# andrewjong/SwapNet

Hardware: NVIDIA H100
Metric: images/sec (G+D fwd+bwd) warp-stage 512x512 (higher is better)
Workload: dtype fp16/bf16-split x3 tensor-core products, fp32 accumulate (fp32-faithful)

## Files before the change

swapnet_b200/csrc/gemm_tc.cu:

```cuda
#include "common.cuh"
#include "plan.h"

namespace {

constexpr int kBlockM = 128;
constexpr int kTileRing = 4;
constexpr int kTileBytes = 16384;
constexpr int kConsumerWarps = 8;
constexpr int kProducerWarp = kConsumerWarps;
constexpr int kThreads = (kConsumerWarps + 1) * 32;

template <int NSPLIT>
struct Cfg {
  static constexpr int kPlanes = NSPLIT == 3 ? 2 : 1;
  static constexpr int kStages = NSPLIT == 3 ? 3 : 6;
  static constexpr int kStageBytes = kPlanes * 2 * kTileBytes;
  static constexpr int kSmemBytes = kStages * kStageBytes + 1024;
};

__device__ __forceinline__ float apply_act(float v, int act) {
  if (act == SN_ACT_TANH) return tanhf(v);
  return v;
}

__device__ __forceinline__ float quad_col_sum(float v) {
  v += __shfl_xor_sync(0xffffffffu, v, 4);
  v += __shfl_xor_sync(0xffffffffu, v, 8);
  v += __shfl_xor_sync(0xffffffffu, v, 16);
  return v;
}

template <int NSPLIT, int CW, int BN, bool F16>
__global__ void __launch_bounds__(kThreads, 1)
tap_gemm_kernel(const __grid_constant__ TapGemmParams p, const int m_tiles, const int n_tiles, const int total_tiles) {
  const auto tile_coords = [&](int tile, int& mt, int& nt, int& z) {
    nt = tile % n_tiles;
    const int rest = tile / n_tiles;
    mt = rest % m_tiles;
    z = rest / m_tiles;
  };
  using C = Cfg<NSPLIT>;
  extern __shared__ uint8_t smem_raw[];
  __shared__ __align__(8) uint64_t full_bar[C::kStages];
  __shared__ __align__(8) uint64_t empty_bar[C::kStages];
  __shared__ __align__(8) uint64_t tr_full[kTileRing];
  __shared__ __align__(8) uint64_t tr_empty[kTileRing];
  __shared__ int tile_ring[kTileRing];

  const uint32_t smem_base = (smem_u32(smem_raw) + 1023u) & ~1023u;
  uint8_t* smem = smem_raw + (smem_base - smem_u32(smem_raw));
  const int warp = threadIdx.x >> 5;
  const int lane = threadIdx.x & 31;

  constexpr int cw = CW;
  constexpr int tps = 64 / cw;
  const int tpp = p.ntaps / p.nphase;
  const int k_iters = cw == 64 ? tpp * p.chunks : tpp / tps;

  if (threadIdx.x == 0) {
    for (int s = 0; s < C::kStages; ++s) {
      mbar_init(&full_bar[s], 1);
      mbar_init(&empty_bar[s], 2);
    }
    for (int r = 0; r < kTileRing; ++r) {
      mbar_init(&tr_full[r], 1);
      mbar_init(&tr_empty[r], kConsumerWarps);
    }
    mbar_fence_init();
  }
  if (warp == kProducerWarp && lane == 0) {
    for (int pl = 0; pl < C::kPlanes; ++pl) {
      tma_prefetch_desc(&p.tmA[pl]);
      tma_prefetch_desc(&p.tmB[pl]);
    }
  }
  __syncthreads();

  if (warp == kProducerWarp) {
    if (lane == 0) {
      const uint32_t stage_tx = C::kPlanes * (p.a_rows * 128 + p.block_n * 128);
      uint32_t it = 0, tcount = 0;
      for (int tile = blockIdx.x;; ++tcount) {
        const int next = tile < total_tiles ? (int)gridDim.x + atomicAdd(p.tile_counter, 1) : total_tiles;
        const uint32_t slot = tcount % kTileRing, rph = (tcount / kTileRing) & 1;
        mbar_wait(&tr_empty[slot], rph ^ 1);
        tile_ring[slot] = tile < total_tiles ? tile : -1;
        mbar_arrive(&tr_full[slot]);
        if (tile >= total_tiles) break;
        int mt, nt, z;
        tile_coords(tile, mt, nt, z);
        const int ncol0 = nt * p.block_n;
        const int tap0 = z * tpp;
        const int w0 = (mt % p.tiles_w) * p.tw;
        const int h0 = ((mt / p.tiles_w) % p.tiles_h) * p.th;
        const int n0 = (mt / (p.tiles_w * p.tiles_h)) * p.nb;
        for (int k = 0; k < k_iters; ++k, ++it) {
          const uint32_t s = it % C::kStages;
          const uint32_t ph = (it / C::kStages) & 1;
          mbar_wait(&empty_bar[s], ph ^ 1);
          mbar_expect_tx(&full_bar[s], stage_tx);
          uint8_t* st = smem + s * C::kStageBytes;
          if (cw == 64) {
            const int t = k / p.chunks;
            const int ch = k - t * p.chunks;
            const TapDesc tap = p.taps[tap0 + t];
            if (p.a_merged) {
              tma_load_5d(&p.tmA[0], &full_bar[s], st, tap.c_off + ch * 64, w0 + tap.dw, h0 + tap.dh, n0, 0);
            } else {
#pragma unroll
              for (int pl = 0; pl < C::kPlanes; ++pl)
                tma_load_5d(&p.tmA[pl], &full_bar[s], st + pl * kTileBytes, tap.c_off + ch * 64,
                            w0 + tap.dw, tap.hp, h0 + tap.dh, n0);
            }
            if (p.b_merged) {
              tma_load_3d(&p.tmB[0], &full_bar[s], st + C::kPlanes * kTileBytes, tap.kb_off + ch * 64, ncol0, 0);
            } else {
#pragma unroll
              for (int pl = 0; pl < C::kPlanes; ++pl)
                tma_load_2d(&p.tmB[pl], &full_bar[s], st + (C::kPlanes + pl) * kTileBytes,
                            tap.kb_off + ch * 64, ncol0);
            }
          } else {
            constexpr int sub = 128 * cw * 2;
#pragma unroll
            for (int j = 0; j < tps; ++j) {
              const TapDesc tap = p.taps[tap0 + k * tps + j];
#pragma unroll
              for (int pl = 0; pl < C::kPlanes; ++pl)
                tma_load_5d(&p.tmA[pl], &full_bar[s], st + pl * kTileBytes + j * sub, tap.c_off,
                            w0 + tap.dw, tap.hp, h0 + tap.dh, n0);
            }
            const int kb = p.taps[tap0 + k * tps].kb_off;
            if (p.b_merged) {
              tma_load_3d(&p.tmB[0], &full_bar[s], st + C::kPlanes * kTileBytes, kb, ncol0, 0);
            } else {
#pragma unroll
              for (int pl = 0; pl < C::kPlanes; ++pl)
                tma_load_2d(&p.tmB[pl], &full_bar[s], st + (C::kPlanes + pl) * kTileBytes, kb, ncol0);
            }
          }
        }
        tile = next;
      }
    }
  } else {
    const int wg = warp >> 2;
    const int quad = lane & 3;
    const int row0 = wg * 64 + (warp & 3) * 16 + (lane >> 2);
    int w_i[2], h_i[2], n_i[2];
#pragma unroll
    for (int h = 0; h < 2; ++h) {
      const int row = row0 + 8 * h;
      w_i[h] = row % p.tw;
      h_i[h] = (row / p.tw) % p.th;
      n_i[h] = row / (p.tw * p.th);
    }
    const float oscale = p.b_scale ? p.b_scale[1] : 1.f;
    float acc[BN / 2];
    uint32_t it = 0;
    for (uint32_t tcount = 0;; ++tcount) {
      const uint32_t slot = tcount % kTileRing, rph = (tcount / kTileRing) & 1;
      mbar_wait(&tr_full[slot], rph);
      const int tile = tile_ring[slot];
      __syncwarp();
      if (lane == 0) mbar_arrive(&tr_empty[slot]);
      if (tile < 0) break;
      for (int k = 0; k < k_iters; ++k, ++it) {
        const uint32_t s = it % C::kStages;
        const uint32_t ph = (it / C::kStages) & 1;
        mbar_wait(&full_bar[s], ph);
        const uint32_t st = smem_base + s * C::kStageBytes;
        constexpr uint32_t a_layout = cw >= 64 ? 1u : (cw == 32 ? 2u : 3u);
        constexpr uint32_t a_sbo = 8u * cw * 2u;
        const uint32_t a_row0 = (uint32_t)wg * 64u * cw * 2u;
        const uint64_t a_hi = gmma_smem_desc(st + a_row0, 16, a_sbo, a_layout);
        const uint64_t b_hi = gmma_smem_desc(st + C::kPlanes * kTileBytes, 16, 1024);
        const uint64_t a_lo = gmma_smem_desc(st + p.a_lo_off + a_row0, 16, a_sbo, a_layout);
        const uint64_t b_lo = gmma_smem_desc(st + C::kPlanes * kTileBytes + p.b_lo_off, 16, 1024);
        constexpr uint32_t sub16 = (uint32_t)(128 * cw * 2) >> 4;
        wgmma_fence();
#pragma unroll
        for (int kk = 0; kk < 4; ++kk) {
          const uint64_t badv = (uint64_t)(kk * 2);
          const uint64_t aadv = (uint64_t)(((kk * 16) / cw) * sub16 + (((kk * 16) % cw) >> 3));
          Wgmma<BN, F16>::template mma<0, 0>(acc, a_hi + aadv, b_hi + badv, (k | kk) != 0);
          if (NSPLIT == 3) {
            Wgmma<BN, F16>::template mma<0, 0>(acc, a_lo + aadv, b_hi + badv, 1);
            Wgmma<BN, F16>::template mma<0, 0>(acc, a_hi + aadv, b_lo + badv, 1);
          }
        }
        wgmma_commit();
        wgmma_wait<0>();
        wgmma_fence_acc(acc);
        if ((threadIdx.x & 127) == 0) mbar_arrive(&empty_bar[s]);
      }

      int mt, nt, z;
      tile_coords(tile, mt, nt, z);
      const int ncol0 = nt * p.block_n;
      const int ph_h = p.nphase == 4 ? (z >> 1) : 0, ph_w = p.nphase == 4 ? (z & 1) : 0;
      int gw[2], gh[2], gn[2];
      bool valid[2];
      float* optr[2];
#pragma unroll
      for (int h = 0; h < 2; ++h) {
        gw[h] = (mt % p.tiles_w) * p.tw + w_i[h];
        gh[h] = ((mt / p.tiles_w) % p.tiles_h) * p.th + h_i[h];
        gn[h] = (mt / (p.tiles_w * p.tiles_h)) * p.nb + n_i[h];
        valid[h] = (row0 + 8 * h < p.a_rows) && (gw[h] < p.m_w) && (gh[h] < p.m_h) && (gn[h] < p.m_n);
        optr[h] = p.out + (long long)gn[h] * p.out_sn + (long long)(gh[h] * p.omh + p.ooh + ph_h) * p.out_sh +
                  (long long)(gw[h] * p.omw + p.oow + ph_w) * p.out_sw + ncol0;
      }
#pragma unroll
      for (int i = 0; i < BN / 8; ++i) {
        const int c = 8 * i + 2 * quad;
        if (BN > 16 && 8 * i >= p.block_n) break;
        if (p.stack_slot) {
#pragma unroll
          for (int h = 0; h < 2; ++h) {
            if (!valid[h]) continue;
#pragma unroll
            for (int e = 0; e < 2; ++e) {
              const int col = ncol0 + c + e;
              const int ph = col / p.stack_slot, ch = col - ph * p.stack_slot;
              if (ph < 4 && ch < p.stack_c) {
                float v = acc[4 * i + 2 * h + e] * oscale;
                if (p.bias) v += p.bias[ch];
                float* o = p.out + (long long)gn[h] * p.out_sn + (long long)(gh[h] * p.omh + (ph >> 1)) * p.out_sh +
                           (long long)(gw[h] * p.omw + (ph & 1)) * p.out_sw + ch;
                *o = apply_act(v, p.act);
              }
            }
          }
        } else if (p.stats) {
          if (ncol0 + 8 * i >= p.n_valid) continue;
          float v[2][2];
#pragma unroll
          for (int h = 0; h < 2; ++h) {
#pragma unroll
            for (int e = 0; e < 2; ++e) {
              float t = acc[4 * i + 2 * h + e] * oscale;
              if (p.bias) t += p.bias[ncol0 + c + e];
              v[h][e] = valid[h] ? t : 0.f;
            }
            if (valid[h]) *reinterpret_cast<float2*>(optr[h] + c) = make_float2(v[h][0], v[h][1]);
          }
          const float s0 = quad_col_sum(v[0][0] + v[1][0]);
          const float s1 = quad_col_sum(v[0][1] + v[1][1]);
          const float q0 = quad_col_sum(v[0][0] * v[0][0] + v[1][0] * v[1][0]);
          const float q1 = quad_col_sum(v[0][1] * v[0][1] + v[1][1] * v[1][1]);
          if (lane < 4) {
            const int tn = (mt / (p.tiles_w * p.tiles_h)) * p.nb;
            double* sp = p.stats + ((long long)tn * p.n_valid + ncol0 + c) * 2;
            atomicAdd(sp, (double)s0);
            atomicAdd(sp + 1, (double)q0);
            atomicAdd(sp + 2, (double)s1);
            atomicAdd(sp + 3, (double)q1);
          }
        } else {
#pragma unroll
          for (int h = 0; h < 2; ++h) {
            if (!valid[h]) continue;
            float v0 = acc[4 * i + 2 * h] * oscale, v1 = acc[4 * i + 2 * h + 1] * oscale;
            const int col = ncol0 + c;
            if (p.vec4 && col + 1 < p.n_valid) {
              if (p.bias) {
                const float2 bb = *reinterpret_cast<const float2*>(p.bias + col);
                v0 += bb.x; v1 += bb.y;
              }
              *reinterpret_cast<float2*>(optr[h] + c) = make_float2(apply_act(v0, p.act), apply_act(v1, p.act));
            } else {
              if (col < p.n_valid) optr[h][c] = apply_act(p.bias ? v0 + p.bias[col] : v0, p.act);
              if (col + 1 < p.n_valid) optr[h][c + 1] = apply_act(p.bias ? v1 + p.bias[col + 1] : v1, p.act);
            }
          }
        }
      }
    }
  }

  __syncthreads();
  if (threadIdx.x == 0) {
    __threadfence();
    if (atomicAdd(p.tile_counter + 1, 1) == (int)gridDim.x - 1) {
      p.tile_counter[0] = 0;
      p.tile_counter[1] = 0;
      __threadfence();
    }
  }
}

// ... 129 lines not shown
        const int row = row0 + 8 * h;
        if (row >= p.rows_valid) continue;
        float* orow = p.out + (long long)row * p.s_row;
#pragma unroll
        for (int i = 0; i < BN / 8; ++i) {
#pragma unroll
          for (int e = 0; e < 2; ++e) {
            const int c = 8 * i + 2 * quad + e;
            const float v = acc[4 * i + 2 * h + e];
            if (!grouped) {
              const int col = ncol0 + c;
              if (c < p.block_n && col < p.cols_valid) atomicAdd(orow + p.tap_off[tap_i] + (long long)col * p.s_col, v);
            } else {
              const int b = c / ycw;
              const int cbase = c - b * ycw;
              if (b < gsize && cbase < p.cols_valid)
                atomicAdd(orow + p.tap_off[tap_i + b] + (long long)cbase * p.s_col, v);
            }
          }
        }
      }
    }
  }
}

}

typedef CUresult (*PFN_encodeTiled)(CUtensorMap*, CUtensorMapDataType, cuuint32_t, void*,
                                    const cuuint64_t*, const cuuint64_t*, const cuuint32_t*,
                                    const cuuint32_t*, CUtensorMapInterleave, CUtensorMapSwizzle,
                                    CUtensorMapL2promotion, CUtensorMapFloatOOBfill);

static PFN_encodeTiled get_encode_fn() {
  static PFN_encodeTiled fn = nullptr;
  if (!fn) {
    void* ptr = nullptr;
    cudaDriverEntryPointQueryResult qres;
    cudaError_t e = cudaGetDriverEntryPoint("cuTensorMapEncodeTiled", &ptr, cudaEnableDefault, &qres);
    if (e != cudaSuccess || qres != cudaDriverEntryPointSuccess || !ptr) return nullptr;
    fn = reinterpret_cast<PFN_encodeTiled>(ptr);
  }
  return fn;
}

int sn_make_act_map(CUtensorMap* tm, const void* base, int N, int H, int W, int C, int pitch,
                    int parity, int box_w, int box_h, int box_n, int chunk = 64, long long plane_stride = 0) {
  PFN_encodeTiled enc = get_encode_fn();
  SN_REQUIRE(enc != nullptr, "cuTensorMapEncodeTiled driver entry point unavailable");
  SN_REQUIRE(pitch % 8 == 0 && ((uintptr_t)base % 16) == 0,
             "activation plane needs 16-B aligned base and pitch %% 8 == 0 (pitch=%d)", pitch);
  SN_REQUIRE(box_w >= 1 && box_h >= 1 && box_n >= 1 && box_w <= 256 && box_h <= 256 && box_n <= 256,
             "bad TMA box %d x %d x %d", box_w, box_h, box_n);
  cuuint64_t dims[5];
  cuuint64_t strides[4];
  const cuuint64_t e = 2;
  cuuint32_t box[5] = {(cuuint32_t)chunk, (cuuint32_t)box_w, 1, (cuuint32_t)box_h, (cuuint32_t)box_n};
  if (plane_stride > 0) {
    SN_REQUIRE(plane_stride % 16 == 0, "merged planes: 16-B aligned plane stride");
    if (!parity) {
      dims[0] = C; dims[1] = W; dims[2] = H; dims[3] = N; dims[4] = 2;
      strides[0] = (cuuint64_t)pitch * e;
      strides[1] = (cuuint64_t)W * pitch * e;
    } else {
      SN_REQUIRE(H % 2 == 0 && W % 2 == 0, "parity view needs even H, W (got %d x %d)", H, W);
      dims[0] = (cuuint64_t)(W + 1) * pitch + C; dims[1] = W / 2; dims[2] = H / 2; dims[3] = N; dims[4] = 2;
      strides[0] = (cuuint64_t)2 * pitch * e;
      strides[1] = (cuuint64_t)2 * W * pitch * e;
    }
    strides[2] = (cuuint64_t)H * W * pitch * e;
    strides[3] = (cuuint64_t)plane_stride;
    box[2] = (cuuint32_t)box_h; box[3] = (cuuint32_t)box_n; box[4] = 2;
  } else if (!parity) {
    dims[0] = C; dims[1] = W; dims[2] = 1; dims[3] = H; dims[4] = N;
    strides[0] = (cuuint64_t)pitch * e;
    strides[1] = (cuuint64_t)W * pitch * e;
    strides[2] = (cuuint64_t)W * pitch * e;
    strides[3] = (cuuint64_t)H * W * pitch * e;
  } else {
    SN_REQUIRE(H % 2 == 0 && W % 2 == 0, "parity view needs even H, W (got %d x %d)", H, W);
    dims[0] = (cuuint64_t)pitch + C; dims[1] = W / 2; dims[2] = 2; dims[3] = H / 2; dims[4] = N;
    strides[0] = (cuuint64_t)2 * pitch * e;
    strides[1] = (cuuint64_t)W * pitch * e;
    strides[2] = (cuuint64_t)2 * W * pitch * e;
    strides[3] = (cuuint64_t)H * W * pitch * e;
  }
  SN_REQUIRE(chunk == 64 || chunk == 32 || chunk == 16, "row chunk must be 64, 32 or 16 channels (got %d)", chunk);
  cuuint32_t estr[5] = {1, 1, 1, 1, 1};
  const CUtensorMapSwizzle swz = chunk == 64 ? CU_TENSOR_MAP_SWIZZLE_128B
                                 : chunk == 32 ? CU_TENSOR_MAP_SWIZZLE_64B : CU_TENSOR_MAP_SWIZZLE_32B;
  CUresult r = enc(tm, CU_TENSOR_MAP_DATA_TYPE_BFLOAT16, 5, const_cast<void*>(base), dims, strides,
                   box, estr, CU_TENSOR_MAP_INTERLEAVE_NONE, swz,
                   CU_TENSOR_MAP_L2_PROMOTION_L2_256B, CU_TENSOR_MAP_FLOAT_OOB_FILL_NONE);
  SN_REQUIRE(r == CUDA_SUCCESS,
             "cuTensorMapEncodeTiled(act) failed: %d (N=%d H=%d W=%d C=%d pitch=%d parity=%d box=%dx%dx%d)",
             (int)r, N, H, W, C, pitch, parity, box_w, box_h, box_n);
  return SN_OK;
}

int sn_make_weight_map(CUtensorMap* tm, const void* base, int rows, long long k_total, int box_rows,
                       long long plane_stride = 0) {
  PFN_encodeTiled enc = get_encode_fn();
  SN_REQUIRE(enc != nullptr, "cuTensorMapEncodeTiled driver entry point unavailable");
  SN_REQUIRE(k_total % 64 == 0 && ((uintptr_t)base % 16) == 0, "packed weights need K %% 64 == 0");
  cuuint64_t dims[3] = {(cuuint64_t)k_total, (cuuint64_t)rows, 2};
  cuuint64_t strides[2] = {(cuuint64_t)k_total * 2, (cuuint64_t)plane_stride};
  cuuint32_t box[3] = {64, (cuuint32_t)box_rows, 2};
  cuuint32_t estr[3] = {1, 1, 1};
  CUresult r = enc(tm, CU_TENSOR_MAP_DATA_TYPE_BFLOAT16, plane_stride > 0 ? 3 : 2, const_cast<void*>(base), dims, strides,
                   box, estr, CU_TENSOR_MAP_INTERLEAVE_NONE, CU_TENSOR_MAP_SWIZZLE_128B,
                   CU_TENSOR_MAP_L2_PROMOTION_L2_256B, CU_TENSOR_MAP_FLOAT_OOB_FILL_NONE);
  SN_REQUIRE(r == CUDA_SUCCESS, "cuTensorMapEncodeTiled(weights) failed: %d (rows=%d K=%lld box_rows=%d)",
             (int)r, rows, k_total, box_rows);
  return SN_OK;
}

static void pick_patch(int m_h, int m_w, int rows, int* th, int* tw, int* nb) {
  int w = 16;
  while (w > 1 && w / 2 >= m_w) w /= 2;
  if (w > rows) w = rows;
  int h = rows / w;
  while (h > 1 && h / 2 >= m_h) h /= 2;
  *tw = w;
  *th = h;
  *nb = rows / (w * h);
}

static void pick_patch_conv(int m_n, int m_h, int m_w, int* th, int* tw, int* nb) {
  double best_eff = -1.0;
  int best_perim = 1 << 30, best_rows = 0, best_area = 0;
  const long long useful = (long long)m_n * m_h * m_w;
  for (int w = 1; w <= m_w && w <= 128; ++w) {
    for (int h = 1; h <= m_h && h * w <= 128; ++h) {
      int n = 1;
      if (m_h * m_w < 128) {
        if (w != m_w || h != m_h) continue;
        n = 128 / (w * h);
        if (n > m_n) n = m_n;
        if (n > 256) n = 256;
      }
      const long long tiles = (long long)((m_w + w - 1) / w) * ((m_h + h - 1) / h) * ((m_n + n - 1) / n);
      const double eff = (double)useful / (double)(tiles * 128);
      const int rows = w * h * n, perim = w + h, area = w * h;
      const bool better =
          eff > best_eff + 1e-9 ||
          (eff > best_eff - 1e-9 &&
           (rows > best_rows ||
            (rows == best_rows && (area > best_area || (area == best_area && (perim < best_perim || (perim == best_perim && w > *tw)))))));
      if (better) {
        best_eff = eff; best_rows = rows; best_perim = perim; best_area = area;
        *tw = w; *th = h; *nb = n;
      }
    }
  }
}

int sn_tap_gemm_plan_init(TapGemmPlan* plan, const sn_tap_gemm_desc* d) {
  memset(plan, 0, sizeof(*plan));
  TapGemmParams& p = plan->p;
  SN_REQUIRE(d->nsplit == 1 || d->nsplit == 3, "nsplit must be 1 or 3");
  SN_REQUIRE(d->ntaps >= 1 && d->ntaps <= SN_MAX_TAPS, "ntaps out of range: %d", d->ntaps);
  const int a_chunk = d->a_chunk ? d->a_chunk : 64;
  SN_REQUIRE(a_chunk == 64 || a_chunk == 32 || a_chunk == 16, "a_chunk must be 64, 32 or 16");
  if (a_chunk == 64) {
    SN_REQUIRE(d->k_per_tap > 0 && d->k_per_tap % 64 == 0, "k_per_tap must be a multiple of 64");
  } else {
    SN_REQUIRE(d->k_per_tap == a_chunk && d->ntaps % (64 / a_chunk) == 0,
               "narrow operand: k_per_tap must equal a_chunk (%d) and ntaps (%d) be a multiple of %d", a_chunk,
               d->ntaps, 64 / a_chunk);
  }
  p.a_chunk = a_chunk;
  SN_REQUIRE(d->block_n >= 16 && d->block_n <= 128 && d->block_n % 16 == 0,
             "block_n must be a multiple of 16 in [16,128]");
  SN_REQUIRE(d->a_hi && d->b_hi && d->out, "null operand");
  SN_REQUIRE(d->nsplit == 1 || (d->a_lo && d->b_lo), "nsplit=3 needs lo planes");
  SN_REQUIRE(d->a_fmt == d->b_fmt, "A and B of one wgmma must share a 16-bit format (a=%d b=%d)",
             d->a_fmt, d->b_fmt);
  int th, tw, nb;
  pick_patch_conv(d->m_n, d->m_h, d->m_w, &th, &tw, &nb);
  p.a_rows = th * tw * nb;
  p.tw = tw; p.th = th; p.nb = nb;
  p.tiles_w = (d->m_w + tw - 1) / tw;
  p.tiles_h = (d->m_h + th - 1) / th;
  p.tiles_n = (d->m_n + nb - 1) / nb;
  p.m_w = d->m_w; p.m_h = d->m_h; p.m_n = d->m_n;
  p.ntaps = d->ntaps;
  p.chunks = a_chunk == 64 ? d->k_per_tap / 64 : 1;
  for (int t = 0; t < d->ntaps; ++t) {
    p.taps[t].c_off = d->taps[t].c_off;
    p.taps[t].kb_off = d->taps[t].kb_off;
    p.taps[t].dw = (short)d->taps[t].dw;
    p.taps[t].dh = (short)d->taps[t].dh;
    p.taps[t].hp = (short)d->taps[t].hp;
  }
  p.block_n = d->block_n;
  p.n_valid = d->n_valid;
  p.out = d->out;
  p.out_sn = d->out_sn; p.out_sh = d->out_sh; p.out_sw = d->out_sw;
  p.omh = d->out_mul_h; p.ooh = d->out_off_h; p.omw = d->out_mul_w; p.oow = d->out_off_w;
  p.nphase = d->nphase == 4 ? 4 : 1;
  SN_REQUIRE(d->nphase == 0 || d->nphase == 1 || d->nphase == 4, "nphase must be 1 or 4");
  if (p.nphase == 4) {
    SN_REQUIRE(d->ntaps % 4 == 0, "4-phase launch: ntaps must split into 4 equal groups");
    const int tpp = d->ntaps / 4;
    SN_REQUIRE(a_chunk == 64 || tpp % (64 / a_chunk) == 0, "4-phase launch: taps per phase must fill whole stages");
  }
  p.bias = d->bias;
  p.stack_slot = d->stack_slot; p.stack_c = d->stack_c;
  p.stats = nullptr;
  if (d->stack_slot > 0)
    SN_REQUIRE(d->nphase <= 1 && d->n_valid == 4 * d->stack_slot && d->stack_c >= 1 && d->stack_c <= d->stack_slot &&
                   d->out_mul_h == 2 && d->out_mul_w == 2,
               "phase-stacked output: n_valid = 4*stack_slot, nphase 1, out_mul 2 (slot=%d c=%d n_valid=%d)",
               d->stack_slot, d->stack_c, d->n_valid);
  p.b_scale = d->b_scale;
  p.a_fmt = d->a_fmt;
  p.b_fmt = d->b_fmt;
  p.act = d->act;
  p.vec4 = ((uintptr_t)d->out % 16 == 0) && (d->out_sn % 4 == 0) && (d->out_sh % 4 == 0) &&
           (d->out_sw % 4 == 0) && (!d->bias || (uintptr_t)d->bias % 16 == 0);
  if (d->stats && nb == 1 && p.vec4 && d->n_valid % 16 == 0 && d->act == 0 && d->stack_slot == 0 && d->m_n * 1 >= 1)
    p.stats = d->stats;
  plan->stats_bytes = p.stats ? sizeof(double) * 2 * (size_t)d->m_n * d->n_valid : 0;
  p.tile_counter = nullptr;
  SN_CHECK_CUDA(cudaMalloc(&p.tile_counter, 2 * sizeof(int)));
  SN_CHECK_CUDA(cudaMemset(p.tile_counter, 0, 2 * sizeof(int)));
  int rc;
  const void* a_pl[2] = {d->a_hi, d->a_lo};
  const void* b_pl[2] = {d->b_hi, d->b_lo};
  const long long a_ps = d->nsplit == 3 ? (const char*)d->a_lo - (const char*)d->a_hi : 0;
  const long long b_ps = d->nsplit == 3 ? (const char*)d->b_lo - (const char*)d->b_hi : 0;
  p.a_merged = a_chunk == 64 && a_ps > 0 && a_ps % 16 == 0 && p.a_rows % 8 == 0;
  if (p.a_merged && d->a_parity)
    for (int t = 0; t < d->ntaps; ++t) p.taps[t].c_off += p.taps[t].hp * d->a_w * d->a_pitch;
  p.b_merged = b_ps > 0 && b_ps % 16 == 0 && d->block_n % 8 == 0;
  p.a_lo_off = p.a_merged ? p.a_rows * 128 : kTileBytes;
  p.b_lo_off = p.b_merged ? d->block_n * 128 : kTileBytes;
  for (int pl = 0; pl < (d->nsplit == 3 ? 2 : 1); ++pl) {
    if (!(p.a_merged && pl == 1)) {
      rc = sn_make_act_map(&p.tmA[pl], a_pl[pl], d->a_n, d->a_h, d->a_w, d->a_c, d->a_pitch,
                           d->a_parity, tw, th, nb, a_chunk, p.a_merged ? a_ps : 0);
      if (rc) return rc;
    }
    if (!(p.b_merged && pl == 1)) {
      rc = sn_make_weight_map(&p.tmB[pl], b_pl[pl], d->b_rows, d->b_k, d->block_n, p.b_merged ? b_ps : 0);
      if (rc) return rc;
    }
  }
  if (p.a_merged) p.tmA[1] = p.tmA[0];
  if (p.b_merged) p.tmB[1] = p.tmB[0];
  plan->nsplit = d->nsplit;
  plan->grid = dim3(p.tiles_w * p.tiles_h * p.tiles_n, (d->n_valid + d->block_n - 1) / d->block_n, p.nphase);
  return SN_OK;
}

static int mma_n(int block_n) {
  return block_n <= 16 ? 16 : block_n <= 32 ? 32 : block_n <= 64 ? 64 : block_n <= 96 ? 96 : 128;
}

template <int NSPLIT, int CW, int BN, bool F16>
static int launch_tap(const TapGemmPlan* plan, cudaStream_t stream) {
  static bool attr_done = false;
  if (!attr_done) {
    SN_CHECK_CUDA(cudaFuncSetAttribute(tap_gemm_kernel<NSPLIT, CW, BN, F16>, cudaFuncAttributeMaxDynamicSharedMemorySize,
                                       Cfg<NSPLIT>::kSmemBytes));
    attr_done = true;
  }
  static int sms = 0;
  if (sms == 0) {
    int dev = 0;
    SN_CHECK_CUDA(cudaGetDevice(&dev));
    SN_CHECK_CUDA(cudaDeviceGetAttribute(&sms, cudaDevAttrMultiProcessorCount, dev));
  }
  const int m_tiles = (int)plan->grid.x, n_tiles = (int)plan->grid.y;
  const int total = m_tiles * n_tiles * (int)plan->grid.z;
  if (plan->p.stats) SN_CHECK_CUDA(cudaMemsetAsync(plan->p.stats, 0, plan->stats_bytes, stream));
  const int ctas = total < sms ? total : sms;
  tap_gemm_kernel<NSPLIT, CW, BN, F16>
      <<<ctas, kThreads, Cfg<NSPLIT>::kSmemBytes, stream>>>(plan->p, m_tiles, n_tiles, total);
  SN_CHECK_CUDA(cudaGetLastError());
  return SN_OK;
}

template <int NSPLIT, int CW, bool F16>
static int launch_tap_n(const TapGemmPlan* plan, cudaStream_t stream) {
  switch (mma_n(plan->p.block_n)) {
    case 16: return launch_tap<NSPLIT, CW, 16, F16>(plan, stream);
    case 32: return launch_tap<NSPLIT, CW, 32, F16>(plan, stream);
    case 64: return launch_tap<NSPLIT, CW, 64, F16>(plan, stream);
    case 96: return launch_tap<NSPLIT, CW, 96, F16>(plan, stream);
    default: return launch_tap<NSPLIT, CW, 128, F16>(plan, stream);
  }
}

template <int NSPLIT, bool F16>
static int launch_tap_cw(const TapGemmPlan* plan, cudaStream_t stream) {
  const int cw = plan->p.a_chunk;
  if (cw == 64) return launch_tap_n<NSPLIT, 64, F16>(plan, stream);
  if (cw == 32) return launch_tap_n<NSPLIT, 32, F16>(plan, stream);
  return launch_tap_n<NSPLIT, 16, F16>(plan, stream);
}

int sn_tap_gemm_plan_launch(const TapGemmPlan* plan, cudaStream_t stream) {
  const bool f16 = plan->p.a_fmt == SN_FMT_F16;
  if (plan->nsplit == 3) return f16 ? launch_tap_cw<3, true>(plan, stream) : launch_tap_cw<3, false>(plan, stream);
  return f16 ? launch_tap_cw<1, true>(plan, stream) : launch_tap_cw<1, false>(plan, stream);
}

int sn_wgrad_plan_init(WgradPlan* plan, const sn_wgrad_desc* d, int sm_count) {
  memset(plan, 0, sizeof(*plan));
  WgradParams& p = plan->p;
  SN_REQUIRE(d->nsplit == 1 || d->nsplit == 3, "nsplit must be 1 or 3");
  SN_REQUIRE(d->ntaps >= 1 && d->ntaps <= SN_MAX_TAPS, "ntaps out of range: %d", d->ntaps);
  const int y_chunk = d->y_chunk ? d->y_chunk : 64;
  SN_REQUIRE(y_chunk == 64 || y_chunk == 32 || y_chunk == 16, "y_chunk must be 64, 32 or 16");
  p.y_chunk = y_chunk;
  p.ngroups = 0;
  int grid_y = d->ntaps;
  if (y_chunk == 64) {
    SN_REQUIRE(d->block_n == 64 || d->block_n == 128, "wgrad block_n must be 64 or 128 for 64-channel Y rows");
  } else {
    SN_REQUIRE(d->cols_valid <= y_chunk, "narrow Y: cols_valid must fit one %d-channel block", y_chunk);
    if (d->ngroups > 0) {
      int maxg = 0, covered = 0;
      for (int g = 0; g < d->ngroups; ++g) {
        SN_REQUIRE(d->group_size[g] >= 1 && d->group_start[g] >= 0 &&
                       d->group_start[g] + d->group_size[g] <= d->ntaps, "bad tap group %d", g);
        if (d->group_size[g] > maxg) maxg = d->group_size[g];
        covered += d->group_size[g];
        p.gstart[g] = (short)d->group_start[g];
        p.gsize[g] = (short)d->group_size[g];
      }
      SN_REQUIRE(covered == d->ntaps && maxg * y_chunk <= 128 && d->block_n == maxg * y_chunk,
                 "tap groups must cover all taps and block_n == max group * y_chunk <= 128");
      p.ngroups = d->ngroups;
      grid_y = d->ngroups;
    } else {
      SN_REQUIRE(d->block_n == y_chunk, "narrow Y without groups: block_n must equal y_chunk");
    }
  }
  SN_REQUIRE(d->x_hi && d->y_hi && d->out, "null operand");
  SN_REQUIRE(d->nsplit == 1 || (d->x_lo && d->y_lo), "nsplit=3 needs lo planes");
  SN_REQUIRE(d->x_fmt == d->y_fmt, "X and Y of one wgmma must share a 16-bit format (x=%d y=%d)",
             d->x_fmt, d->y_fmt);
  int th, tw, nb;
  pick_patch(d->m_h, d->m_w, 64, &th, &tw, &nb);
  p.tw = tw; p.th = th; p.nb = nb;
  p.tiles_w = (d->m_w + tw - 1) / tw;
  p.tiles_h = (d->m_h + th - 1) / th;
  p.tiles_n = (d->m_n + nb - 1) / nb;
  p.ntaps = d->ntaps;
  for (int t = 0; t < d->ntaps; ++t) {
    p.xtaps[t].c_off = d->xtaps[t].c_off; p.xtaps[t].dw = (short)d->xtaps[t].dw;
    p.xtaps[t].dh = (short)d->xtaps[t].dh; p.xtaps[t].hp = (short)d->xtaps[t].hp;
    p.ytaps[t].c_off = d->ytaps[t].c_off; p.ytaps[t].dw = (short)d->ytaps[t].dw;
    p.ytaps[t].dh = (short)d->ytaps[t].dh; p.ytaps[t].hp = (short)d->ytaps[t].hp;
    p.tap_off[t] = d->tap_off[t];
  }
  p.block_n = d->block_n;
  p.m_tiles = (d->rows_valid + kBlockM - 1) / kBlockM;
  p.n_tiles = y_chunk == 64 ? (d->cols_valid + d->block_n - 1) / d->block_n : 1;
  p.rows_valid = d->rows_valid;
  p.cols_valid = d->cols_valid;
  p.out = d->out;
  p.s_row = d->s_row;
  p.s_col = d->s_col;
  p.x_fmt = d->x_fmt;
  p.y_fmt = d->y_fmt;
  int rc;
  const void* x_pl[2] = {d->x_hi, d->x_lo};
  const void* y_pl[2] = {d->y_hi, d->y_lo};
  {
    const long long x_ps = d->nsplit == 3 ? (const char*)d->x_lo - (const char*)d->x_hi : 0;
    const long long y_ps = d->nsplit == 3 ? (const char*)d->y_lo - (const char*)d->y_hi : 0;
    p.x_merged = x_ps > 0 && x_ps % 16 == 0 && tw * th * nb == 64;
    p.y_merged = y_ps > 0 && y_ps % 16 == 0 && tw * th * nb == 64 && y_chunk == 64 && d->ngroups == 0;
    for (int t = 0; t < d->ntaps; ++t) {
      if (p.x_merged && d->x_parity) p.xtaps[t].c_off += p.xtaps[t].hp * d->x_w * d->x_pitch;
      if (p.y_merged && d->y_parity) p.ytaps[t].c_off += p.ytaps[t].hp * d->y_w * d->y_pitch;
    }
    for (int pl = 0; pl < (d->nsplit == 3 ? 2 : 1); ++pl) {
      if (!(p.x_merged && pl == 1)) {
        rc = sn_make_act_map(&p.tmX[pl], x_pl[pl], d->x_n, d->x_h, d->x_w, d->x_c, d->x_pitch,
                             d->x_parity, tw, th, nb, 64, p.x_merged ? x_ps : 0);
        if (rc) return rc;
      }
      if (!(p.y_merged && pl == 1)) {
        rc = sn_make_act_map(&p.tmY[pl], y_pl[pl], d->y_n, d->y_h, d->y_w, d->y_c, d->y_pitch,
                             d->y_parity, tw, th, nb, y_chunk, p.y_merged ? y_ps : 0);
        if (rc) return rc;
      }
    }
    if (p.x_merged) p.tmX[1] = p.tmX[0];
    if (p.y_merged) p.tmY[1] = p.tmY[0];
  }
  plan->nsplit = d->nsplit;
  const int base_ctas = p.m_tiles * p.n_tiles * grid_y;
  const int total = p.tiles_w * p.tiles_h * p.tiles_n;
  int ks = d->ksplit;
  if (ks <= 0) {
    ks = (3 * sm_count + base_ctas - 1) / base_ctas;
    int max_ks = total / 8;
    if (max_ks < 1) max_ks = 1;
    if (ks > max_ks) ks = max_ks;
    if (ks < 1) ks = 1;
  }
  if (ks > total) ks = total;
  plan->grid = dim3(p.m_tiles * p.n_tiles, grid_y, ks);
  return SN_OK;
}

template <int NSPLIT, int BN, bool F16>
static int launch_wgrad(const WgradPlan* plan, cudaStream_t stream) {
  static bool attr_done = false;
  if (!attr_done) {
    SN_CHECK_CUDA(cudaFuncSetAttribute(wgrad_gemm_kernel<NSPLIT, BN, F16>, cudaFuncAttributeMaxDynamicSharedMemorySize,
                                       Cfg<NSPLIT>::kSmemBytes));
    attr_done = true;
  }
  wgrad_gemm_kernel<NSPLIT, BN, F16><<<plan->grid, kThreads, Cfg<NSPLIT>::kSmemBytes, stream>>>(plan->p);
  SN_CHECK_CUDA(cudaGetLastError());
  return SN_OK;
}

template <int NSPLIT, bool F16>
static int launch_wgrad_n(const WgradPlan* plan, cudaStream_t stream) {
  switch (mma_n(plan->p.block_n)) {
    case 16: return launch_wgrad<NSPLIT, 16, F16>(plan, stream);
    case 32: return launch_wgrad<NSPLIT, 32, F16>(plan, stream);
    case 64: return launch_wgrad<NSPLIT, 64, F16>(plan, stream);
    case 96: return launch_wgrad<NSPLIT, 96, F16>(plan, stream);
    default: return launch_wgrad<NSPLIT, 128, F16>(plan, stream);
// ... 9 lines not shown
```

swapnet_b200/lowering.py:

```python
from __future__ import annotations

from dataclasses import dataclass, field
from typing import List, Tuple

KINDS = ("conv4s2", "convT4s2", "conv3r", "conv4s1", "head", "conv3z")

@dataclass
class Tap:
    pw: int
    kb: int
    dw: int
    dh: int
    hp: int = 0


@dataclass
class GemmSpec:
    parity: bool
    m_h: int
    m_w: int
    taps: List[Tap]
    out_mul: Tuple[int, int] = (1, 1)
    out_off: Tuple[int, int] = (0, 0)
    w_phase: int = 0
# ... 69 lines not shown
    if kind == "conv4s2":
        taps = []
        for kh in range(4):
            dh, hp = _s2_tap(kh)
            for kw in range(4):
                dw, pw = _s2_tap(kw)
                taps.append(Tap(pw, kh * 4 + kw, dw, dh, hp))
        return [GemmSpec(True, h // 2, w // 2, taps, a_hw=(h, w))]
    if kind == "convT4s2":
        slot = phase_major_slots()
        return [GemmSpec(False, h, w, [Tap(0, slot[kh * 4 + kw], dw, dh) for kh, dh, kw, dw in taps], (2, 2),
                         (py, px), a_hw=(h, w)) for (py, px), taps in _phase_taps()]
    if kind == "conv3r":
        taps = [Tap(0, kh * 3 + kw, kw, kh) for kh in range(3) for kw in range(3)]
        return [GemmSpec(False, h, w, taps, a_hw=(h + 2, w + 2))]
    if kind == "conv4s1":
        taps = [Tap(0, kh * 4 + kw, kw - 1, kh - 1) for kh in range(4) for kw in range(4)]
        return [GemmSpec(False, h - 1, w - 1, taps, a_hw=(h, w))]
    if kind == "conv3z":
        taps = [Tap(0, kh * 3 + kw, kw - 1, kh - 1) for kh in range(3) for kw in range(3)]
        return [GemmSpec(False, h, w, taps, a_hw=(h, w))]
    if kind == "head":
        specs = []
        for py in range(2):
            for px in range(2):
                taps = []
                for ey in range(head_neff(py)):
                    for ex in range(head_neff(px)):
                        taps.append(Tap(0, ey * head_neff(px) + ex, ex - 1, ey - 1))
                specs.append(GemmSpec(False, h, w, taps, (2, 2), (py, px), w_phase=2 * py + px, a_hw=(h, w)))
        return specs
    raise ValueError(kind)


HEAD_SLOT = 24


def head_stacked_spec(h: int, w: int) -> GemmSpec:
    taps = [Tap(0, (sy + 1) * 3 + (sx + 1), sx, sy) for sy in (-1, 0, 1) for sx in (-1, 0, 1)]
    return GemmSpec(False, h, w, taps, (2, 2), (0, 0), a_hw=(h, w))


def dgrad_specs(kind: str, h: int, w: int) -> List[GemmSpec]:
    oh, ow = out_hw(kind, h, w)
    if kind == "conv4s2":
        slot = phase_major_slots()
        return [GemmSpec(False, oh, ow, [Tap(0, slot[kh * 4 + kw], dw, dh) for kh, dh, kw, dw in taps], (2, 2),
                         (py, px), a_hw=(oh, ow)) for (py, px), taps in _phase_taps()]
    if kind == "convT4s2":
        taps = []
        for kh in range(4):
            dh, hp = _s2_tap(kh)
            for kw in range(4):
                dw, pw = _s2_tap(kw)
                taps.append(Tap(pw, kh * 4 + kw, dw, dh, hp))
        return [GemmSpec(True, h, w, taps, a_hw=(oh, ow))]
    if kind == "conv3r":
        taps = [Tap(0, kh * 3 + kw, -kw, -kh) for kh in range(3) for kw in range(3)]
        return [GemmSpec(False, h + 2, w + 2, taps, a_hw=(oh, ow))]
    if kind == "conv4s1":
        taps = [Tap(0, kh * 4 + kw, 1 - kw, 1 - kh) for kh in range(4) for kw in range(4)]
        return [GemmSpec(False, h, w, taps, a_hw=(oh, ow))]
    if kind == "conv3z":
        taps = [Tap(0, kh * 3 + kw, 1 - kw, 1 - kh) for kh in range(3) for kw in range(3)]
        return [GemmSpec(False, h, w, taps, a_hw=(oh, ow))]
    if kind == "head":
        taps = []
        for py in range(2):
            for px in range(2):
                for ey in range(head_neff(py)):
                    for ex in range(head_neff(px)):
                        te = HEAD_PHASE_OFF[2 * py + px] + ey * head_neff(px) + ex
                        taps.append(Tap(px, te, -(ex - 1), -(ey - 1), py))
        return [GemmSpec(True, h, w, taps, a_hw=(oh, ow))]
    raise ValueError(kind)


def wgrad_specs(kind: str, h: int, w: int) -> List[WgradSpec]:
    oh, ow = out_hw(kind, h, w)
    zero = Tap(0, 0, 0, 0, 0)
    if kind == "conv4s2":
        yt = []
        for kh in range(4):
            dh, hp = _s2_tap(kh)
            for kw in range(4):
                dw, pw = _s2_tap(kw)
                yt.append(Tap(pw, 0, dw, dh, hp))
        return [WgradSpec(oh, ow, False, True, [zero] * 16, yt, "dy", list(range(16)))]
    if kind == "convT4s2":
        yt = []
        for kh in range(4):
            dh, hp = _s2_tap(kh)
            for kw in range(4):
                dw, pw = _s2_tap(kw)
                yt.append(Tap(pw, 0, dw, dh, hp))
        return [WgradSpec(h, w, False, True, [zero] * 16, yt, "in", list(range(16)))]
    if kind == "conv3r":
        yt = [Tap(0, 0, kw, kh) for kh in range(3) for kw in range(3)]
        return [WgradSpec(h, w, False, False, [zero] * 9, yt, "dy", list(range(9)))]
    if kind == "conv4s1":
        yt = [Tap(0, 0, kw - 1, kh - 1) for kh in range(4) for kw in range(4)]
        return [WgradSpec(oh, ow, False, False, [zero] * 16, yt, "dy", list(range(16)))]
    if kind == "conv3z":
        yt = [Tap(0, 0, kw - 1, kh - 1) for kh in range(3) for kw in range(3)]
        return [WgradSpec(oh, ow, False, False, [zero] * 9, yt, "dy", list(range(9)))]
    if kind == "head":
        xt, yt, ids = [], [], []
        for py in range(2):
            for px in range(2):
                for ey in range(head_neff(py)):
                    for ex in range(head_neff(px)):
                        xt.append(Tap(px, 0, 0, 0, py))
                        yt.append(Tap(0, 0, ex - 1, ey - 1))
                        ids.append(HEAD_PHASE_OFF[2 * py + px] + ey * head_neff(px) + ex)
        return [WgradSpec(h, w, True, False, xt, yt, "dy", ids)]
    raise ValueError(kind)


def pack_strides(kind: str, cin: int, cout: int, dgrad: bool) -> Tuple[int, int, int, int]:
    t = ntaps(kind)
    if kind == "convT4s2":
        if not dgrad:
            return t, cout * t, cout, cin
        return cout * t, t, cin, cout
    if not dgrad:
        return cin * t, t, cout, cin
    return t, cin * t, cin, cout


def wgrad_out_strides(kind: str, cin: int, cout: int, x_is_dy: bool) -> Tuple[int, int]:
    t = ntaps(kind)
    if kind == "head":
        co_s, ci_s = 25 * cin, 1
    elif kind == "convT4s2":
        ci_s, co_s = cout * t, t
    else:
        co_s, ci_s = cin * t, t
    return (co_s, ci_s) if x_is_dy else (ci_s, co_s)


def pad64(c: int) -> int:
    return (c + 63) // 64 * 64


def padc(c: int) -> int:
    if c <= 16:
        return 16
    if c <= 32:
        return 32
    return pad64(c)


def pick_block_n(n_valid: int) -> int:
    if n_valid >= 128:
        return 128
    for b in (16, 32, 64, 128):
        if n_valid <= b:
            return b
    return 128
```

swapnet_b200/ops.py:

```python
from __future__ import annotations

import ctypes as C
from dataclasses import dataclass
from typing import Optional, Sequence, Tuple

import torch

from . import _lib
from . import lowering as L

from ._lib import (ACT_LRELU, ACT_NONE, ACT_RELU, ACT_TANH, FMT_BF16, FMT_F16, LAYOUT_LABEL_U8, LAYOUT_MASK_I32,
                   LAYOUT_NCHW, LAYOUT_NHWC, SnGradSrc, SnNormActBwdDesc, SnNormActDesc, SnTap, SnTapGemmDesc,
                   SnWgradDesc, check)

IN_EPS = 1e-5


def _stream() -> int:
    return torch.cuda.current_stream().cuda_stream


def _ptr(t: Optional[torch.Tensor]) -> Optional[int]:
    return None if t is None else t.data_ptr()


class Planes:

    def __init__(self, n: int, h: int, w: int, pitch: int, device, c: Optional[int] = None, c_off: int = 0,
                 hi: Optional[torch.Tensor] = None, lo: Optional[torch.Tensor] = None, fmt: int = FMT_F16,
                 dual: bool = False, twin: Optional["Planes"] = None):
        assert pitch % 8 == 0
        self.fmt = fmt
        self.twin = twin
        if dual and twin is None:
            self.twin = Planes(n, h, w, pitch, device, c, c_off, fmt=FMT_BF16)
        self.n, self.h, self.w, self.pitch = n, h, w, pitch
        self.c = pitch if c is None else c
        self.c_off = c_off
        if hi is None:
            assert lo is None
            buf = torch.zeros(2, n, h, w, pitch, dtype=torch.bfloat16, device=device)
            hi, lo = buf[0], buf[1]
        self.hi, self.lo = hi, lo

    def slice(self, c_off: int, c: int) -> "Planes":
        assert c_off + c <= self.pitch
        return Planes(self.n, self.h, self.w, self.pitch, self.hi.device, c, self.c_off + c_off, self.hi, self.lo,
                      self.fmt, twin=None if self.twin is None else self.twin.slice(c_off, c))

    def batch_slice(self, n0: int, n: int) -> "Planes":
        return Planes(n, self.h, self.w, self.pitch, self.hi.device, self.c, self.c_off, self.hi[n0:n0 + n],
                      self.lo[n0:n0 + n], self.fmt, twin=None if self.twin is None else self.twin.batch_slice(n0, n))

    @property
    def hi_ptr(self) -> int:
        return self.hi.data_ptr() + 2 * self.c_off

    @property
    def lo_ptr(self) -> int:
        return self.lo.data_ptr() + 2 * self.c_off

    def dense(self) -> torch.Tensor:
        s = slice(self.c_off, self.c_off + self.c)
        if self.fmt == FMT_F16:
            return self.hi[..., s].view(torch.float16).float() + self.lo[..., s].view(torch.float16).float()
        return self.hi[..., s].float() + self.lo[..., s].float()


class PackedWeights:

    def __init__(self, rows: int, k_total: int, device, scale: Optional[torch.Tensor] = None, fmt: int = FMT_F16):
        self.rows, self.k_total = rows, k_total
        self.fmt = fmt
        self.scale = scale if (scale is not None and fmt == FMT_F16) else None
        buf = torch.zeros(2, rows, k_total, dtype=torch.bfloat16, device=device)
        self.hi, self.lo = buf[0], buf[1]


class Plan:

    def __init__(self, handle: int, keep: Sequence, tag=None):
        self.handle = handle
        self.tag = tag
        self._keep = list(keep)

    @property
    def has_stats(self) -> bool:
        return bool(_lib.load().sn_plan_has_stats(self.handle))

    trace = None

    def run(self) -> None:
        if Plan.trace is None:
            check(_lib.load().sn_plan_run(self.handle, _stream()))
            return
        e0, e1 = torch.cuda.Event(enable_timing=True), torch.cuda.Event(enable_timing=True)
        e0.record()
        check(_lib.load().sn_plan_run(self.handle, _stream()))
        e1.record()
        Plan.trace.append((self, e0, e1))

    def __del__(self):
        try:
            if self.handle:
                _lib.load().sn_plan_destroy(self.handle)
        except Exception:
            pass


def _fill_tap(dst: SnTap, tap: L.Tap, pitch: int, k_pad: int, c_base: int = 0) -> None:
    dst.c_off = tap.pw * pitch + c_base
    dst.kb_off = tap.kb * k_pad
    dst.dw, dst.dh, dst.hp = tap.dw, tap.dh, tap.hp


def tap_gemm_desc(a: Planes, spec: L.GemmSpec, w: PackedWeights, k_per_tap: int, out: torch.Tensor,
                  n_valid: int, *, w_row_off: int = 0, w_rows: Optional[int] = None,
                  w_k: Optional[int] = None, w_elem_off: int = 0, bias: Optional[torch.Tensor] = None,
                  act: int = ACT_NONE, nsplit: int = 3, block_n: Optional[int] = None,
                  out_c_off: int = 0, nphase: int = 1, stack_slot: int = 0, stack_c: int = 0,
                  stats: Optional[torch.Tensor] = None) -> SnTapGemmDesc:
    assert (a.h, a.w) == tuple(spec.a_hw), f"operand is {a.h}x{a.w}, spec wants {spec.a_hw}"
    assert a.c_off % 8 == 0 and k_per_tap <= a.c
    narrow = k_per_tap < 64
    assert (k_per_tap in (16, 32)) if narrow else (k_per_tap % 64 == 0)
    taps = list(spec.taps)
    if narrow and nphase == 4:
        assert (len(taps) // 4) % (64 // k_per_tap) == 0, "4-phase narrow launch: taps per phase must fill whole stages"
    elif narrow:
        tps = 64 // k_per_tap
        kb_next = max(t.kb for t in taps) + 1
        while len(taps) % tps:
            taps.append(L.Tap(taps[0].pw, kb_next, taps[0].dw, taps[0].dh, taps[0].hp))
            kb_next += 1
    d = SnTapGemmDesc()
    d.a_chunk = k_per_tap if narrow else 64
    d.a_hi, d.a_lo = a.hi_ptr, a.lo_ptr
    d.a_n, d.a_h, d.a_w, d.a_c, d.a_pitch = a.n, a.h, a.w, a.c, a.pitch
    d.a_parity = 1 if spec.parity else 0
    d.a_fmt, d.b_fmt = a.fmt, w.fmt
    d.b_scale = None if w.scale is None else w.scale.data_ptr()
    d.b_hi = w.hi.data_ptr() + 2 * w_elem_off
    d.b_lo = w.lo.data_ptr() + 2 * w_elem_off
    d.b_rows = w.rows if w_rows is None else w_rows
    d.b_k = w.k_total if w_k is None else w_k
    d.m_n, d.m_h, d.m_w = a.n, spec.m_h, spec.m_w
    d.ntaps, d.k_per_tap = len(taps), k_per_tap
    for i, t in enumerate(taps):
        _fill_tap(d.taps[i], t, a.pitch, k_per_tap)
    assert out.dtype == torch.float32 and out.dim() == 4 and (out.shape[3] == 1 or out.stride(3) == 1)
    d.out = out.data_ptr() + 4 * out_c_off
    d.out_sn, d.out_sh, d.out_sw = out.stride(0), out.stride(1), out.stride(2)
    d.out_mul_h, d.out_mul_w = spec.out_mul
    d.out_off_h, d.out_off_w = spec.out_off
    d.n_valid = n_valid
    d.block_n = block_n or L.pick_block_n(n_valid)
    d.bias = _ptr(bias)
    d.act = act
    d.nsplit = nsplit
    d.nphase = nphase
    d.stack_slot, d.stack_c = stack_slot, stack_c
    if stats is not None:
        assert stats.dtype == torch.float64 and stats.numel() >= a.n * n_valid * 2 and out_c_off == 0
        d.stats = stats.data_ptr()
    return d


def merge_phase_specs(specs) -> Optional[L.GemmSpec]:
    if len(specs) != 4:
        return None
    s0 = specs[0]
    n = len(s0.taps)
    for z, s in enumerate(specs):
        if (s.parity, s.m_h, s.m_w, s.out_mul, s.a_hw, len(s.taps)) != (s0.parity, s0.m_h, s0.m_w, s0.out_mul, s0.a_hw, n):
            return None
        if s.out_off != (z >> 1, z & 1) or s.w_phase != 0:
            return None
    return L.GemmSpec(s0.parity, s0.m_h, s0.m_w, [t for s in specs for t in s.taps], s0.out_mul, (0, 0), 0, s0.a_hw)


def tap_gemm_plan(desc: SnTapGemmDesc, keep: Sequence = ()) -> Plan:
    h = C.c_void_p()
    check(_lib.load().sn_tap_gemm_plan_create(C.byref(desc), C.byref(h)))
    return Plan(h.value, keep)


def tap_gemm_simt(desc: SnTapGemmDesc) -> None:
    check(_lib.load().sn_tap_gemm_simt(C.byref(desc), _stream()))


def wgrad_desc(x: Planes, y: Planes, spec: L.WgradSpec, out: torch.Tensor, s_row: int, s_col: int,
               tap_off: Sequence[int], rows_valid: int, cols_valid: int, *, swap: bool = False,
               nsplit: int = 3, block_n: Optional[int] = None, ksplit: int = 0) -> SnWgradDesc:
    xt, yt = spec.xtaps, spec.ytaps
    xp, yp = spec.x_parity, spec.y_parity
    if swap:
        x, y, xt, yt, xp, yp = y, x, yt, xt, yp, xp
        s_row, s_col = s_col, s_row
        rows_valid, cols_valid = cols_valid, rows_valid
    assert x.c_off % 8 == 0 and y.c_off % 8 == 0
    order = list(range(len(xt)))
    groups = []
    if y.c < 64:
        gmax = 128 // y.c
        key = lambda i: (xt[i].pw, xt[i].dw, xt[i].dh, xt[i].hp)
        order = sorted(order, key=key)
        i = 0
        while i < len(order):
            j = i
            while j < len(order) and j - i < gmax and key(order[j]) == key(order[i]):
                j += 1
            groups.append((i, j - i))
            i = j
        xt = [xt[i] for i in order]
        yt = [yt[i] for i in order]
        tap_off = [tap_off[i] for i in order]
    d = SnWgradDesc()
    d.x_hi, d.x_lo = x.hi_ptr, x.lo_ptr
    d.x_n, d.x_h, d.x_w, d.x_c, d.x_pitch, d.x_parity = x.n, x.h, x.w, x.c, x.pitch, int(xp)
    d.x_fmt, d.y_fmt = x.fmt, y.fmt
    d.y_hi, d.y_lo = y.hi_ptr, y.lo_ptr
    d.y_n, d.y_h, d.y_w, d.y_c, d.y_pitch, d.y_parity = y.n, y.h, y.w, y.c, y.pitch, int(yp)
    d.m_n, d.m_h, d.m_w = x.n, spec.m_h, spec.m_w
    d.ntaps = len(xt)
    for i in range(len(xt)):
        _fill_tap(d.xtaps[i], xt[i], x.pitch, 0)
        _fill_tap(d.ytaps[i], yt[i], y.pitch, 0)
        d.tap_off[i] = tap_off[i]
    assert out.dtype == torch.float32
    d.out = out.data_ptr()
    d.s_row, d.s_col = s_row, s_col
    d.rows_valid, d.cols_valid = rows_valid, cols_valid
    assert x.c >= 64, "the 128-row operand of a wgrad GEMM must carry >= 64 channels (swap the roles)"
    if y.c < 64:
        assert y.c in (16, 32) and cols_valid <= y.c
        d.y_chunk = y.c
        d.ngroups = len(groups)
        for g, (st, sz) in enumerate(groups):
            d.group_start[g], d.group_size[g] = st, sz
        d.block_n = max(sz for _, sz in groups) * y.c
    else:
        d.y_chunk = 64
        d.block_n = block_n or (128 if cols_valid > 64 else 64)
    d.ksplit = ksplit
    d.nsplit = nsplit
    return d


def wgrad_plan(desc: SnWgradDesc, keep: Sequence = ()) -> Plan:
    h = C.c_void_p()
    check(_lib.load().sn_wgrad_plan_create(C.byref(desc), C.byref(h)))
    return Plan(h.value, keep)


class SegMap:

    def __init__(self, data: torch.Tensor, channels: int):
        assert data.dim() == 3 and data.dtype in (torch.uint8, torch.int32), "uint8 label map or int32 bit mask [n,h,w]"
        assert channels <= (32 if data.dtype == torch.int32 else 256)
        self.data, self.channels = data.contiguous(), channels
        self.layout = LAYOUT_LABEL_U8 if data.dtype == torch.uint8 else LAYOUT_MASK_I32

    @property
    def shape(self):
        n, h, w = self.data.shape
        return (n, self.channels, h, w)

    @property
    def is_cuda(self):
        return self.data.is_cuda

    def dense(self) -> torch.Tensor:
        ch = torch.arange(self.channels, device=self.data.device).view(1, -1, 1, 1)
        d = self.data.unsqueeze(1)
        if self.layout == LAYOUT_LABEL_U8:
            return ((d.long() == ch) & (ch > 0)).float()
        return ((d.long() >> ch) & 1).float()

    @staticmethod
    def from_dense(t: torch.Tensor) -> "SegMap":
        assert t.dim() == 4 and t.shape[1] <= 32
        b = t != 0
        if not torch.equal(b.to(t.dtype), t):
            raise ValueError("SegMap.from_dense: tensor is not 0/1-valued")
        c = t.shape[1]
        if int(b.sum(1).max()) <= 1 and not bool(b[:, 0].any()):
            return SegMap(b.to(torch.uint8).mul(torch.arange(c, dtype=torch.uint8, device=t.device).view(1, -1, 1, 1))
                          .sum(1, dtype=torch.uint8), c)
        w = (1 << torch.arange(c, dtype=torch.int64, device=t.device)).view(1, -1, 1, 1)
        return SegMap((b.long() * w).sum(1).to(torch.int32), c)


def _src_args(t, nhwc: bool):
    if isinstance(t, SegMap):
        n, h, w = t.data.shape
        return t.data.data_ptr(), t.layout, 0, t.channels, (n, h, w)
    assert t.dtype == torch.float32
    if nhwc:
        n, h, w, c = t.shape
        return t.data_ptr(), LAYOUT_NHWC, _pitch(t), c, (n, h, w)
    assert t.is_contiguous()
    n, c, h, w = t.shape
    return t.data_ptr(), LAYOUT_NCHW, 0, c, (n, h, w)


def pack_planes(src, dst: Planes, *, nhwc: bool = False) -> None:
    if isinstance(src, SegMap):
        ptr, layout, _, c, (n, h, w) = _src_args(src, False)
        assert c <= dst.c and (n, h, w) == (dst.n, dst.h, dst.w)
        for d_ in ((dst,) if dst.twin is None else (dst, dst.twin)):
            check(_lib.load().sn_pack_planes(ptr, layout, 0, n, c, h, w, d_.hi_ptr, d_.lo_ptr, d_.pitch, 0, d_.fmt,
                                             _stream()))
        return
    assert src.dtype == torch.float32
    if nhwc:
        n, h, w, sp = src.shape
        assert src.stride(3) == 1 and src.stride(2) == sp
        c = dst.c
        for d_ in ((dst,) if dst.twin is None else (dst, dst.twin)):
            check(_lib.load().sn_pack_planes(src.data_ptr(), LAYOUT_NHWC, sp, n, c, h, w, d_.hi_ptr, d_.lo_ptr,
                                             d_.pitch, 0, d_.fmt, _stream()))
    else:
        assert src.is_contiguous()
        n, c, h, w = src.shape
        assert c <= dst.c
        for d_ in ((dst,) if dst.twin is None else (dst, dst.twin)):
            check(_lib.load().sn_pack_planes(src.data_ptr(), LAYOUT_NCHW, 0, n, c, h, w, d_.hi_ptr, d_.lo_ptr,
                                             d_.pitch, 0, d_.fmt, _stream()))
    assert (n, h, w) == (dst.n, dst.h, dst.w)


def pack_concat(srcs, dst: Planes) -> None:
    assert 1 <= len(srcs) <= 2 and dst.c % 8 == 0 and dst.c_off % 8 == 0
    args = []
    for t, nhwc in srcs:
        ptr, layout, pitch, c, nhw = _src_args(t, nhwc)
        args += [ptr, layout, pitch, c]
# ... 513 lines not shown
```

Baseline: 138.8.

## Size tap GEMM pipeline stages by block_n and allow 96-wide N tiles

Shared-memory stage size is now computed from the actual B tile width (BN*128 bytes per plane), not a fixed 16 KB, so narrow-N split-precision configs fit more pipeline stages within the shared-memory budget. B plane offsets and b_lo_off are updated to match the tighter packing. pick_block_n now picks 96 over 128 when n_valid > 128 and 96 wastes fewer padded columns. It also records k_stages on Python plans, which has no speed effect. The deeper pipeline adds barriers and shared memory, and 96-wide tiles may map less evenly onto the MMA shape.

```diff
diff --git a/swapnet_b200/csrc/gemm_tc.cu b/swapnet_b200/csrc/gemm_tc.cu
--- a/swapnet_b200/csrc/gemm_tc.cu
+++ b/swapnet_b200/csrc/gemm_tc.cu
@@ -16,6 +16,18 @@
   static constexpr int kStages = NSPLIT == 3 ? 3 : 6;
   static constexpr int kStageBytes = kPlanes * 2 * kTileBytes;
   static constexpr int kSmemBytes = kStages * kStageBytes + 1024;
+};
+
+constexpr int kSmemBudget = 227 * 1024 - 2048;
+template <int NSPLIT, int BN>
+struct TapCfg {
+  static constexpr int kPlanes = NSPLIT == 3 ? 2 : 1;
+  static constexpr int kBPlaneBytes = BN * 128;
+  static constexpr int kStageBytes = kPlanes * (kTileBytes + kBPlaneBytes);
+  static constexpr int kStages = NSPLIT == 3 ? (kSmemBudget - 1024) / kStageBytes : 6;
+  static constexpr int kSmemBytes = kStages * kStageBytes + 1024;
+  static_assert(kStages >= 3 && kSmemBytes <= kSmemBudget, "tap GEMM stages do not fit shared memory");
+  static_assert(kStageBytes % 1024 == 0, "stages must keep the 1024-B alignment of the 128B swizzle");
 };
 
 __device__ __forceinline__ float apply_act(float v, int act) {
@@ -39,7 +51,7 @@
     mt = rest % m_tiles;
     z = rest / m_tiles;
   };
-  using C = Cfg<NSPLIT>;
+  using C = TapCfg<NSPLIT, BN>;
   extern __shared__ uint8_t smem_raw[];
   __shared__ __align__(8) uint64_t full_bar[C::kStages];
   __shared__ __align__(8) uint64_t empty_bar[C::kStages];
@@ -117,7 +129,7 @@
             } else {
 #pragma unroll
               for (int pl = 0; pl < C::kPlanes; ++pl)
-                tma_load_2d(&p.tmB[pl], &full_bar[s], st + (C::kPlanes + pl) * kTileBytes,
+                tma_load_2d(&p.tmB[pl], &full_bar[s], st + C::kPlanes * kTileBytes + pl * C::kBPlaneBytes,
                             tap.kb_off + ch * 64, ncol0);
             }
           } else {
@@ -136,7 +148,8 @@
             } else {
 #pragma unroll
               for (int pl = 0; pl < C::kPlanes; ++pl)
-                tma_load_2d(&p.tmB[pl], &full_bar[s], st + (C::kPlanes + pl) * kTileBytes, kb, ncol0);
+                tma_load_2d(&p.tmB[pl], &full_bar[s], st + C::kPlanes * kTileBytes + pl * C::kBPlaneBytes, kb,
+                            ncol0);
             }
           }
         }
@@ -572,6 +585,10 @@
       }
     }
   }
+}
+
+static int mma_n(int block_n) {
+  return block_n <= 16 ? 16 : block_n <= 32 ? 32 : block_n <= 64 ? 64 : block_n <= 96 ? 96 : 128;
 }
 
 int sn_tap_gemm_plan_init(TapGemmPlan* plan, const sn_tap_gemm_desc* d) {
@@ -654,7 +671,7 @@
     for (int t = 0; t < d->ntaps; ++t) p.taps[t].c_off += p.taps[t].hp * d->a_w * d->a_pitch;
   p.b_merged = b_ps > 0 && b_ps % 16 == 0 && d->block_n % 8 == 0;
   p.a_lo_off = p.a_merged ? p.a_rows * 128 : kTileBytes;
-  p.b_lo_off = p.b_merged ? d->block_n * 128 : kTileBytes;
+  p.b_lo_off = p.b_merged ? d->block_n * 128 : mma_n(d->block_n) * 128;
   for (int pl = 0; pl < (d->nsplit == 3 ? 2 : 1); ++pl) {
     if (!(p.a_merged && pl == 1)) {
       rc = sn_make_act_map(&p.tmA[pl], a_pl[pl], d->a_n, d->a_h, d->a_w, d->a_c, d->a_pitch,
@@ -673,16 +690,12 @@
   return SN_OK;
 }
 
-static int mma_n(int block_n) {
-  return block_n <= 16 ? 16 : block_n <= 32 ? 32 : block_n <= 64 ? 64 : block_n <= 96 ? 96 : 128;
-}
-
 template <int NSPLIT, int CW, int BN, bool F16>
 static int launch_tap(const TapGemmPlan* plan, cudaStream_t stream) {
   static bool attr_done = false;
   if (!attr_done) {
     SN_CHECK_CUDA(cudaFuncSetAttribute(tap_gemm_kernel<NSPLIT, CW, BN, F16>, cudaFuncAttributeMaxDynamicSharedMemorySize,
-                                       Cfg<NSPLIT>::kSmemBytes));
+                                       TapCfg<NSPLIT, BN>::kSmemBytes));
     attr_done = true;
   }
   static int sms = 0;
@@ -696,7 +709,7 @@
   if (plan->p.stats) SN_CHECK_CUDA(cudaMemsetAsync(plan->p.stats, 0, plan->stats_bytes, stream));
   const int ctas = total < sms ? total : sms;
   tap_gemm_kernel<NSPLIT, CW, BN, F16>
-      <<<ctas, kThreads, Cfg<NSPLIT>::kSmemBytes, stream>>>(plan->p, m_tiles, n_tiles, total);
+      <<<ctas, kThreads, TapCfg<NSPLIT, BN>::kSmemBytes, stream>>>(plan->p, m_tiles, n_tiles, total);
   SN_CHECK_CUDA(cudaGetLastError());
   return SN_OK;
 }
diff --git a/swapnet_b200/lowering.py b/swapnet_b200/lowering.py
--- a/swapnet_b200/lowering.py
+++ b/swapnet_b200/lowering.py
@@ -245,9 +245,8 @@
 
 
 def pick_block_n(n_valid: int) -> int:
-    if n_valid >= 128:
-        return 128
-    for b in (16, 32, 64, 128):
-        if n_valid <= b:
-            return b
-    return 128
+    if n_valid <= 128:
+        for b in (16, 32, 64, 128):
+            if n_valid <= b:
+                return b
+    return min((128, 96), key=lambda b: -(-n_valid // b) * b)
diff --git a/swapnet_b200/ops.py b/swapnet_b200/ops.py
--- a/swapnet_b200/ops.py
+++ b/swapnet_b200/ops.py
@@ -83,6 +83,7 @@
         self.handle = handle
         self.tag = tag
         self._keep = list(keep)
+        self.k_stages = None
 
     @property
     def has_stats(self) -> bool:
@@ -179,10 +180,18 @@
     return L.GemmSpec(s0.parity, s0.m_h, s0.m_w, [t for s in specs for t in s.taps], s0.out_mul, (0, 0), 0, s0.a_hw)
 
 
+def tap_k_stages(desc: SnTapGemmDesc) -> int:
+    tpp = desc.ntaps // (4 if desc.nphase == 4 else 1)
+    chunk = desc.a_chunk or 64
+    return tpp * (desc.k_per_tap // 64) if chunk == 64 else tpp // (64 // chunk)
+
+
 def tap_gemm_plan(desc: SnTapGemmDesc, keep: Sequence = ()) -> Plan:
     h = C.c_void_p()
     check(_lib.load().sn_tap_gemm_plan_create(C.byref(desc), C.byref(h)))
-    return Plan(h.value, keep)
+    plan = Plan(h.value, keep)
+    plan.k_stages = tap_k_stages(desc)
+    return plan
 
 
 def tap_gemm_simt(desc: SnTapGemmDesc) -> None:
```

Result: no change. 139.4, median of 6 (+0.5%).
